# ishine/chunkformer

Hardware: AMD Instinct MI355X
Metric: audio-frames/sec (80-dim fbank) through encoder, chunkformer-large chunk=64, 1/2/4/8 GPU (higher is better)
Workload: dtype bf16

## Files before the change

chunkformer_amd/csrc/cfm_kernels.h:

```cpp
#pragma once
#include <hip/hip_runtime.h>
#include <stdint.h>

typedef __bf16 bf16;

#define CFM_HD_INLINE __host__ __device__ __forceinline__

namespace cfm {

int cu_count();

enum { EPI_STORE = 0, EPI_STORE_F32 = 1, EPI_RESID = 2, EPI_QKV = 3, EPI_GLU = 4, EPI_DW2 = 5 };
enum { ACT_NONE = 0, ACT_RELU = 1, ACT_SILU = 2, ACT_SILU_L2E = 3 };

struct EpiArgs {
  const float* bias = nullptr;
  float alpha = 1.f;
  void* out = nullptr;
  void* out2 = nullptr;
  int ldo = 0;
  int row_off = 0;
  float* x = nullptr;
  int ldx = 0;
  const uint8_t* rowmask = nullptr;
  int d = 0;
  int dk = 64;
  int col_group = 0;
  int store_mode = 0;
  int diag = 0;
  int wst = 1;
  int small_tiles = 0;
  int big_min_tiles = 0;
  int wsp_small_div = 1;
  int wsp_small_rows = 32768;
  int f16 = 0;
  const float* dw_w = nullptr;
  const float* dw_b = nullptr;
  int t2n = 0, t3n = 0;
};

int gemm_bf16_wst(int epi, int act, const bf16* A, int lda, const bf16* W, int ldw, int M, int N, int K,
                  const EpiArgs& ep, hipStream_t st);

enum { SITE_QKV = 1, SITE_OPROJ = 2, SITE_PW2 = 4, SITE_FFN2 = 8, SITE_FFN1 = 16, SITE_PW1 = 32, SITE_FE = 64 };

struct Tuning {
  int gemm_diag = 0, gemm_wst = 1, store_mode = 0, col_group = 0;
  int dw2_seg = 4;
  int fe_conv = 6;
  int fe_fuse_dw2 = 1;
  int nt_sites = 8;
  int big_min_tiles = 0;
  int wsp_small_div = 1;
  int wsp_small_rows = 32768;
  int attn_min_chunks = 2;
  void apply(EpiArgs& e, int site = 0) const {
    e.diag = gemm_diag;
    e.big_min_tiles = big_min_tiles;
    e.wsp_small_div = wsp_small_div;
    e.wsp_small_rows = wsp_small_rows;
    e.wst = gemm_wst;
    e.store_mode = (nt_sites & site) ? 2 : store_mode;
    e.col_group = col_group;
  }
};

template <typename T>
int gemm(int epi, int act, const T* A, int lda, const T* W, int ldw, int M, int N, int K, const EpiArgs& ep,
         hipStream_t st);

template <typename T>
inline int vocab_logits(const T* A, int rows, const T* W, const float* bias, int V, int d, float* out, int ldo,
                        hipStream_t st, const EpiArgs& tuned = EpiArgs()) {
  const int V1 = (sizeof(T) == 2 && V % 4 == 0) ? V / 256 * 256 : 0;
  if (V1 > 0) {
    EpiArgs e = tuned; e.bias = bias; e.out = out; e.ldo = ldo;
    if (const int r = gemm<T>(EPI_STORE_F32, ACT_NONE, A, d, W, d, rows, V1, d, e, st)) return r;
  }
  if (V1 < V) {
    EpiArgs e = tuned; e.bias = bias + V1; e.out = out + V1; e.ldo = ldo;
    if (const int r = gemm<T>(EPI_STORE_F32, ACT_NONE, A, d, W + (size_t)V1 * d, d, rows, V - V1, d, e, st)) return r;
  }
  return 0;
}
inline int logit_slab_rows(int V) {
  const size_t r = (((size_t)512 << 20) / ((size_t)V * sizeof(float))) / 256 * 256;
  return (int)(r < 256 ? 256 : r > 16384 ? 16384 : r);
}

template <typename T> struct ResidAdd {
  const T* y = nullptr;
  float alpha = 1.f;
  const uint8_t* ymask = nullptr;
  const T* y2 = nullptr;
  float alpha2 = 1.f;
  const uint8_t* ymask2 = nullptr;
  bool defer = false;
};
template <typename T>
int layernorm(float* x, const ResidAdd<T>& ra, int M, int d, const float* w, const float* b, float eps, T* out,
              const uint8_t* rowmask, hipStream_t st);
template <typename T>
int layernorm2(float* x, const ResidAdd<T>& ra, int M, int d, const float* w1, const float* b1, const float* w2,
               const float* b2, float eps, T* out, hipStream_t st);
template <typename T>
int layernorm2_f32(float* x, const ResidAdd<T>& ra, int M, int d, const float* w1, const float* b1, const float* w2,
                   const float* b2, float eps, float* out, hipStream_t st);

template <typename T>
int chunk_attention(const T* q, const T* kv, int kv_rows, const T* P, int p_rows, const float* pos_u,
                    const float* pos_v, const int32_t* desc, int nblk, int H, int dk, T* out, hipStream_t st,
                    int p_ld = 0);

CFM_HD_INLINE int qkv_kv_col(int cc, int which, int dk) { return (cc / dk) * 2 * dk + which * dk + (cc & (dk - 1)); }

int full_attention_bf16(const bf16* q, const bf16* kv, int kv_rows, const bf16* P, int p_rows, const float* pos_u,
                        const float* pos_v, const int32_t* desc, int nutt, int nd, int H, int dk, int t_keys,
                        bf16* out, hipStream_t st, int p_ld);
int chunk_attention_masked_bf16(const bf16* q, const bf16* kv, int kv_rows, const bf16* P, int p_rows,
                                const float* pos_u, const float* pos_v, const int32_t* desc, int n_chunks, int H,
                                int C, int W, bf16* out, hipStream_t st, int diag = 0, int p_ld = 0,
                                int min_chunks = 2);
int chunk_attention_masked_f16(const f16* q, const f16* kv, int kv_rows, const f16* P, int p_rows,
                               const float* pos_u, const float* pos_v, const int32_t* desc, int n_chunks, int H,
                               int C, int W, f16* out, hipStream_t st, int diag = 0, int p_ld = 0,
                               int min_chunks = 2);

bool attention_a128_eligible(int C, int W, int p_rows, int dk);
int vt_transpose_bf16(const bf16* kv, int kv_rows, int H, bf16* vt, int vt_ld, hipStream_t st);
int chunk_attention_masked_a128(const bf16* q, const bf16* kv, int kv_rows, const bf16* vt, int vt_ld, const bf16* P,
                                int p_rows, int p_ld, const float* pos_u, const float* pos_v, const int32_t* desc,
                                int n_chunks, int H, int C, int W, bf16* out, hipStream_t st);

template <typename T>
int conv_dw_ln_silu(const T* glu, const int32_t* desc, int nblk, int d, const float* wdw_t ,
                    const float* bdw, const float* lnw, const float* lnb, float eps, T* out, hipStream_t st);

template <typename T>
int frontend_conv0_dw(const float* feats, const float* const* tab, int step, const int32_t* meta, int meta_stride,
                      int nwin, int W,
                      const float* cmvn_mean, const float* cmvn_istd, const float* w0, const float* b0,
                      const float* w1, const float* b1, const float* wpack, const float* wfrag, int d, T* out,
                      hipStream_t st, int var = 1);
constexpr int FE_WPACK = 24;
constexpr int FE2_NFRAG = 23;
template <typename T>
int frontend_dw2(const T* in, int nwin, int T2, int d, const float* w, const float* b, T* out, hipStream_t st,
                 int seg = 4);

template <typename T>
int pos_table(int d, int p_rows, int anchor, T* out, hipStream_t st);
template <typename T>
int att_cache_in(const float* cache, int L, int row_elems, T* kv, hipStream_t st);
template <typename T>
int att_cache_out(const T* kv, int start_row, int L, int row_elems, float* cache, hipStream_t st);
template <typename T>
int att_cache_in_hl(const float* cache , int H, int L, int dk, T* kv, hipStream_t st);
template <typename T>
int att_cache_out_hl(const T* kv, int start_row, int H, int L, int dk, float* cache , hipStream_t st);
template <typename T>
int cnn_cache_in(const float* cache , int d, int lorder, T* glu, hipStream_t st);
template <typename T>
int cnn_cache_out(const T* glu, int start_row, int d, int lorder, float* cache, hipStream_t st);
template <typename T>
int cache_io(bool in, bool hl, float* acache, int H, int L, int dk, T* kv, float* ccache, int d, int lorder, T* glu,
             hipStream_t st);
int masks_from_plan(const int32_t* meta, int n, int C, int L, int R, uint8_t* att, uint8_t* pad, hipStream_t st);
bool ctc_argmax_eligible(int V, int d);
int ctc_argmax_bf16(const float* enc, int M, const bf16* W, const float* bias, int V, int d, int32_t* ids,
                    hipStream_t st);
int ctc_argmax_f16(const float* enc, int M, const f16* W, const float* bias, int V, int d, int32_t* ids,
                   hipStream_t st);
int ctc_collapse(const int32_t* ids, const int32_t* row_start, const int32_t* row_len, int B, int blank, int max_sil,
                 int32_t* tok, int32_t* tok_frame, int32_t* n_tok, int32_t* seg, int32_t* n_seg, hipStream_t st);
int log_softmax_rows(float* logits, int M, int V, int write_logp, int32_t* ids, hipStream_t st);
int ctc_topk_rows(const float* x, int M, int V, int k, int with_lse, float* vals, int32_t* ids, hipStream_t st);

}
```

chunkformer_amd/csrc/frontend.hip:

```cpp
#include <algorithm>
#include <cstdlib>
#include <type_traits>
#include "cfm_common.h"
#include "cfm_kernels.h"

namespace cfm {

constexpr int FE_T2_TILE = 8;
constexpr int FE_T1_ROWS = 2 * FE_T2_TILE + 1;
constexpr int FE_IN_ROWS = 2 * FE_T1_ROWS + 1;
constexpr int FE_F0 = 80, FE_F1 = 39, FE_F2 = 19, FE_F3 = 9;
constexpr int FE_CG = 16;

__device__ __forceinline__ const float* window_rows(const float* feats, const float* const* tab, int step,
                                                   const int32_t* m) {
  return tab ? tab[m[PM_UTT]] + (size_t)m[PM_CHUNK] * step * FE_F0 : feats + (size_t)m[PM_SRC_ROW] * FE_F0;
}

template <typename T>
__global__ __launch_bounds__(256) void fe_conv0_dw_kernel(const float* __restrict__ feats, const float* const* __restrict__ tab,
                                                          int step, const int32_t* __restrict__ meta,
                                                          int meta_stride, int W, int T2, const float* __restrict__ cm,
                                                          const float* __restrict__ ci, const float* __restrict__ w0,
                                                          const float* __restrict__ b0, const float* __restrict__ w1,
// ... 65 lines not shown
template <typename E, typename V>
CFM_DEV f32x16 mfma32x16(const V& a, const V& b, const f32x16& c) {
  if constexpr (std::is_same<E, f16>::value) return __builtin_amdgcn_mfma_f32_32x32x16_f16(a, b, c, 0, 0, 0);
  else return __builtin_amdgcn_mfma_f32_32x32x16_bf16(a, b, c, 0, 0, 0);
}
template <typename E>
__global__ __launch_bounds__(256, 3) void fe_conv0_dw_mfma_kernel(const float* __restrict__ feats,
                                                               const float* const* __restrict__ tab, int step,
                                                               const int32_t* __restrict__ meta, int meta_stride,
                                                               int W, int T2, const float* __restrict__ cm,
                                                               const float* __restrict__ ci,
                                                               const float* __restrict__ wpack, int d,
                                                               E* __restrict__ out) {
  typedef E ex8 __attribute__((ext_vector_type(8)));
  __shared__ float xin[FE_XROWS * FE_F0];
  constexpr int OPITCH = 144;
  __shared__ __attribute__((aligned(16))) char ostage[4][32 * OPITCH];
  const int tid = threadIdx.x;
  const int win = blockIdx.y;
  const int P = T2 * FE_F2;
  const int p0 = blockIdx.x * FE_POS_BLOCK;
  const int r0 = 4 * (p0 / FE_F2);
  const float* xsrc = window_rows(feats, tab, step, meta + (size_t)win * meta_stride);
  const int nvalid = min(meta[(size_t)win * meta_stride + PM_NVALID], W);
  for (int idx = tid; idx < FE_XROWS * FE_F0; idx += 256) {
    const int r = idx / FE_F0, f = idx - r * FE_F0, gr = r0 + r;
    float v = gr < nvalid ? xsrc[(size_t)gr * FE_F0 + f] : 0.f;
    if (cm) v = (v - cm[f]) * ci[f];
    xin[idx] = v;
  }
  __syncthreads();
  const int lane = tid & 63, wv = tid >> 6, hh = lane >> 5, n = lane & 31;
  const int pw = p0 + wv * 32;
  if (pw >= P) return;
  ex8 xa[9];
  {
    const int pos = min(pw + n, P - 1);
    const int t2 = pos / FE_F2, f2 = pos - t2 * FE_F2;
    const float* xb = xin + (4 * t2 - r0) * FE_F0 + 4 * f2;
#pragma unroll
    for (int s = 0; s < 9; ++s) {
      const float* xs = xb + 2 * (s / 3) * FE_F0 + 2 * (s % 3);
      if (hh == 0) {
#pragma unroll
        for (int j = 0; j < 8; ++j) xa[s][j] = (E)xs[(j / 3) * FE_F0 + j % 3];
      } else {
        xa[s][0] = (E)xs[2 * FE_F0 + 2];
        xa[s][1] = (E)1.f;
#pragma unroll
        for (int j = 2; j < 8; ++j) xa[s][j] = (E)0.f;
      }
    }
  }
  f32x4 qw[5];
  auto load_w = [&](int c) {
    const f32x4* wp = reinterpret_cast<const f32x4*>(wpack + (size_t)c * FE_WPACK);
#pragma unroll
    for (int i = 0; i < 5; ++i) qw[i] = wp[i];
  };
  load_w(n);
  const unsigned long long obase = (unsigned long long)(out + (size_t)win * P * d);
  const unsigned long long obu = ((unsigned long long)__builtin_amdgcn_readfirstlane((unsigned)(obase >> 32)) << 32) |
                                 (unsigned)__builtin_amdgcn_readfirstlane((unsigned)obase);
  const __amdgpu_buffer_rsrc_t ors = __builtin_amdgcn_make_buffer_rsrc(
      (void*)obu, (short)0, __builtin_amdgcn_readfirstlane(P * d * 2), 0x00020000);
  unsigned voff[4];
#pragma unroll
  for (int k = 0; k < 4; ++k) voff[k] = (unsigned)(((pw + (lane >> 3) + 8 * k) * d + (lane & 7) * 8) * 2);
  for (int ct = 0; ct < d; ct += 64) {
#pragma unroll
    for (int half = 0; half < 2; ++half) {
      const float t[9] = {qw[0][0], qw[0][1], qw[0][2], qw[0][3], qw[1][0], qw[1][1], qw[1][2], qw[1][3], qw[2][0]};
      ex8 wcur;
#pragma unroll
      for (int j = 0; j < 8; ++j) wcur[j] = (E)(hh ? (j == 0 ? t[8] : j == 1 ? qw[4][2] : 0.f) : t[j]);
      const float wkc[9] = {qw[2][1], qw[2][2], qw[2][3], qw[3][0], qw[3][1], qw[3][2], qw[3][3], qw[4][0], qw[4][1]};
      const f32x16 seed = {};
      f32x16 o;
#pragma unroll
      for (int r = 0; r < 16; ++r) o[r] = qw[4][3];
      load_w(min(ct + 32 * half + 32 + n, d - 1));
      f32x16 acc = mfma32x16<E>(xa[0], wcur, seed);
#pragma unroll
      for (int s = 0; s < 9; ++s) {
        f32x16 nxt;
        if (s + 1 < 9) nxt = mfma32x16<E>(xa[s + 1], wcur, seed);
        __builtin_amdgcn_sched_barrier(0);
#pragma unroll
        for (int r = 0; r < 16; ++r) o[r] = fmaf(fmaxf(acc[r], 0.f), wkc[s], o[r]);
        __builtin_amdgcn_sched_barrier(0);
        if (s + 1 < 9) acc = nxt;
      }
      char* os = ostage[wv];
#pragma unroll
      for (int r = 0; r < 16; ++r) {
        const int m = 8 * (r >> 2) + 4 * hh + (r & 3);
        *reinterpret_cast<E*>(os + m * OPITCH + (32 * half + n) * 2) = (E)o[r];
      }
    }
    const char* os = ostage[wv];
#pragma unroll
    for (int k = 0; k < 4; ++k) {
      const u32x4 v = *reinterpret_cast<const u32x4*>(os + ((lane >> 3) + 8 * k) * OPITCH + (lane & 7) * 16);
#ifndef CFM_FE_DIAG_NOSTORE
      __builtin_amdgcn_raw_buffer_store_b128(v, ors, voff[k], ct * 2, 0);
#else
      asm volatile("" ::"v"(v));
#endif
    }
  }
}

constexpr int FE2_WAVES = 4;
constexpr int FE2_POS = 256;
constexpr int FE2_T1ROWS = 2 * ((FE_F2 - 1 + FE2_POS - 1) / FE_F2) + 3;
constexpr int FE2_XROWS = 2 * FE2_T1ROWS + 1;
constexpr int FE2_SLOTS = (FE_F1 + 1) / 2;
__host__ __device__ constexpr int fe2_slot(int t1, int i) { return t1 * FE2_SLOTS + (t1 >> 1) * 11 + i; }
constexpr int FE2_PLANE = fe2_slot(FE2_T1ROWS - 1, FE2_SLOTS - 1) + 1;
constexpr int FE2_IMG = 2 * FE2_PLANE * 16;
constexpr int FE2_OPITCH = 80;
constexpr int FE2_NQ = FE2_XROWS * (FE_F0 / 4);
constexpr int FE2_NT = 64 * FE2_WAVES;
constexpr int FE2_QPT = (FE2_NQ + FE2_NT - 1) / FE2_NT;
typedef short short2v __attribute__((ext_vector_type(2)));
typedef float f32x2v __attribute__((ext_vector_type(2)));

template <typename E>
__device__ __forceinline__ unsigned fe2_relu_pk(float a, float b) {
  if constexpr (std::is_same<E, f16>::value) {
    typedef f16 h2v __attribute__((ext_vector_type(2)));
    short2v v = __builtin_bit_cast(short2v, __builtin_convertvector((f32x2v){a, b}, h2v));
    v = __builtin_elementwise_max(v, (short2v){0, 0});
    return __builtin_bit_cast(unsigned, v);
  }
  unsigned u;
  asm("v_cvt_pk_bf16_f32 %0, %1, %2 clamp" : "=v"(u) : "v"(a), "v"(b));
  return u;
}

template <typename E>
__device__ __forceinline__ bf16x8 pk8(float a, float b, float c, float d_, float e, float f, float g, float h) {
  typedef E e8v __attribute__((ext_vector_type(8)));
  return __builtin_bit_cast(bf16x8, (e8v){(E)a, (E)b, (E)c, (E)d_, (E)e, (E)f, (E)g, (E)h});
}
template <typename E>
__device__ __forceinline__ f32x16 fe2_mfma(const bf16x8& a, const bf16x8& b, const f32x16& c) {
  if constexpr (std::is_same<E, f16>::value)
    return __builtin_amdgcn_mfma_f32_32x32x16_f16(__builtin_bit_cast(f16x8, a), __builtin_bit_cast(f16x8, b), c, 0, 0, 0);
  else
    return __builtin_amdgcn_mfma_f32_32x32x16_bf16(a, b, c, 0, 0, 0);
}
template <typename E>
__global__ __launch_bounds__(FE2_NT, 2) void fe_conv0_dw_mfma2_kernel(const float* __restrict__ feats,
                                                                const float* const* __restrict__ tab, int step,
                                                                const int32_t* __restrict__ meta, int meta_stride,
                                                                int W, int T2, const float* __restrict__ cm,
                                                                const float* __restrict__ ci,
                                                                const float* __restrict__ wfrag, int d,
                                                                E* __restrict__ out) {
  __shared__ __attribute__((aligned(16))) char im2col[2 * FE2_IMG];
  constexpr int XBYTES = FE2_XROWS * FE_F0 * 4, OBYTES = FE2_WAVES * 32 * FE2_OPITCH;
  __shared__ __attribute__((aligned(16))) char xstage[XBYTES > OBYTES ? XBYTES : OBYTES];
  __shared__ __attribute__((aligned(16))) float cmvn[2][FE_F0];
  const int tid = threadIdx.x;
  const int lane = tid & 63, wv = tid >> 6, h = lane >> 5, n = lane & 31;
  if (cm && tid < 2 * FE_F0) cmvn[tid / FE_F0][tid % FE_F0] = (tid < FE_F0 ? cm : ci)[tid % FE_F0];
  const int win = blockIdx.z;
  const int P = T2 * FE_F2;
  const int ct = blockIdx.y * FE2_WAVES + wv;
  const bool active = ct * 32 < d;
  bf16x8 a0, a1[9][2];
  f32x16 seed;
  {
    const u32x4* fr = reinterpret_cast<const u32x4*>(wfrag) + (size_t)(active ? ct : 0) * FE2_NFRAG * 64 + lane;
    a0 = __builtin_bit_cast(bf16x8, fr[0]);
#pragma unroll
    for (int s = 0; s < 9; ++s)
#pragma unroll
      for (int t = 0; t < 2; ++t) a1[s][t] = __builtin_bit_cast(bf16x8, fr[(1 + 2 * s + t) * 64]);
#pragma unroll
    for (int i = 0; i < 4; ++i) {
      const f32x4 v = __builtin_bit_cast(f32x4, fr[(19 + i) * 64]);
#pragma unroll
      for (int r = 0; r < 4; ++r) seed[4 * i + r] = v[r];
    }
  }
  const float* xsrc = window_rows(feats, tab, step, meta + (size_t)win * meta_stride);
  const int nvalid = min(meta[(size_t)win * meta_stride + PM_NVALID], W);
  const int nck = (P + FE2_POS - 1) / FE2_POS;
  const int c_beg = (int)((long long)blockIdx.x * nck / gridDim.x), c_end = (int)((long long)(blockIdx.x + 1) * nck / gridDim.x);
  f32x4 pv[FE2_QPT];
  auto prefetch = [&](int c) {
    const int r0 = 4 * ((c * FE2_POS) / FE_F2);
#pragma unroll
    for (int i = 0; i < FE2_QPT; ++i) {
      const int q = tid + FE2_NT * i, r = q / (FE_F0 / 4), gr = r0 + r;
      pv[i] = (f32x4){0.f, 0.f, 0.f, 0.f};
      if (q < FE2_NQ && gr < nvalid)
        pv[i] = *reinterpret_cast<const f32x4*>(xsrc + (size_t)gr * FE_F0 + 4 * (q % (FE_F0 / 4)));
    }
  };
  if (c_beg < c_end) prefetch(c_beg);
  const unsigned long long obase = (unsigned long long)(out + (size_t)win * P * d);
  const unsigned long long obu = ((unsigned long long)__builtin_amdgcn_readfirstlane((unsigned)(obase >> 32)) << 32) |
                                 (unsigned)__builtin_amdgcn_readfirstlane((unsigned)obase);
  const __amdgpu_buffer_rsrc_t ors = __builtin_amdgcn_make_buffer_rsrc(
      (void*)obu, (short)0, __builtin_amdgcn_readfirstlane(P * d * 2), 0x00020000);
  char* sb = xstage + wv * 32 * FE2_OPITCH;
  const f32x16 zero = {};
  for (int c = c_beg; c < c_end; ++c) {
    const int p0 = c * FE2_POS, t2a = p0 / FE_F2;
    __syncthreads();
    {
      float* xs = reinterpret_cast<float*>(xstage);
#pragma unroll
      for (int i = 0; i < FE2_QPT; ++i) {
        const int q = tid + FE2_NT * i;
        if (q < FE2_NQ) {
          f32x4 x = pv[i];
          if (cm) {
            const int f = 4 * (q % (FE_F0 / 4));
            x = (x - *reinterpret_cast<const f32x4*>(&cmvn[0][f])) * *reinterpret_cast<const f32x4*>(&cmvn[1][f]);
          }
          *reinterpret_cast<f32x4*>(xs + 4 * q) = x;
        }
      }
    }
    __syncthreads();
    for (int idx = tid; idx < FE2_T1ROWS * FE2_SLOTS; idx += FE2_NT) {
      const int tl = idx / FE2_SLOTS, i = idx - tl * FE2_SLOTS;
      const float* xr = reinterpret_cast<const float*>(xstage) + (2 * tl) * FE_F0 + 4 * i;
      f32x4 A[3];
      float Ex[3];
#pragma unroll
      for (int a = 0; a < 3; ++a) {
        A[a] = *reinterpret_cast<const f32x4*>(xr + a * FE_F0);
        Ex[a] = i + 1 < FE2_SLOTS ? xr[a * FE_F0 + 4] : 0.f;
      }
      const bf16x8 lo0 = pk8<E>(A[0][0], A[0][1], A[0][2], A[1][0], A[1][1], A[1][2], A[2][0], A[2][1]);
      const bf16x8 hi0 = pk8<E>(A[2][2], 1.f, 0.f, 0.f, 0.f, 0.f, 0.f, 0.f);
      const int s0 = fe2_slot(tl, i) * 16, s1 = (FE2_PLANE + fe2_slot(tl, i)) * 16;
      *reinterpret_cast<bf16x8*>(im2col + s0) = lo0;
      *reinterpret_cast<bf16x8*>(im2col + FE2_IMG + s0) = hi0;
      if (2 * i + 1 < FE_F1) {
        const bf16x8 lo1 = pk8<E>(A[0][2], A[0][3], Ex[0], A[1][2], A[1][3], Ex[1], A[2][2], A[2][3]);
        const bf16x8 hi1 = pk8<E>(Ex[2], 1.f, 0.f, 0.f, 0.f, 0.f, 0.f, 0.f);
        *reinterpret_cast<bf16x8*>(im2col + s1) = lo1;
        *reinterpret_cast<bf16x8*>(im2col + FE2_IMG + s1) = hi1;
      }
    }
    __syncthreads();
    if (c + 1 < c_end) prefetch(c + 1);
    if (!active) continue;
    const int pend = min(p0 + FE2_POS, P);
    auto patch_base = [&](int pt) {
      const int pos = min(pt + n, P - 1);
      const int t2 = pos / FE_F2, f2 = pos - t2 * FE_F2;
      return im2col + h * FE2_IMG + (fe2_slot(2 * (t2 - t2a), 0) + f2) * 16;
    };
    auto tap_off = [](int s) { return (((s % 3) & 1) * FE2_PLANE + fe2_slot(s / 3, 0) + ((s % 3) >> 1)) * 16; };
    auto ld = [&](const char* xb, int s) { return *reinterpret_cast<const bf16x8*>(xb + tap_off(s)); };
    auto flush = [&](const char* sb, int pt) {
#pragma unroll
      for (int k = 0; k < 2; ++k) {
        const int pl = (lane >> 2) + 16 * k, ch = lane & 3;
        const u32x4 v = *reinterpret_cast<const u32x4*>(sb + pl * FE2_OPITCH + ch * 16);
#ifndef CFM_FE_DIAG_NOSTORE
        __builtin_amdgcn_raw_buffer_store_b128(v, ors, (unsigned)(((pt + pl) * d + ct * 32 + ch * 8) * 2), 0, 0);
#else
        asm volatile("" ::"v"(v));
#endif
      }
    };
    bf16x8 pb[9];
    {
      const char* xb = patch_base(p0);
#pragma unroll
      for (int s = 0; s < 9; ++s) pb[s] = ld(xb, s);
    }
    for (int pt = p0; pt < pend; pt += 32) {
      const char* xbn = patch_base(pt + 32 < pend ? pt + 32 : pt);
      f32x16 y = seed;
      f32x16 acc = fe2_mfma<E>(a0, pb[0], zero);
#pragma unroll
      for (int s = 0; s < 9; ++s) {
        f32x16 nxt;
        if (s + 1 < 9) nxt = fe2_mfma<E>(a0, pb[s + 1], zero);
        __builtin_amdgcn_sched_barrier(0);
        u32x4 r0, r1;
#pragma unroll
        for (int q = 0; q < 4; ++q) {
          r0[q] = fe2_relu_pk<E>(acc[2 * q], acc[2 * q + 1]);
          r1[q] = fe2_relu_pk<E>(acc[8 + 2 * q], acc[9 + 2 * q]);
        }
        y = fe2_mfma<E>(a1[s][0], __builtin_bit_cast(bf16x8, r0), y);
        y = fe2_mfma<E>(a1[s][1], __builtin_bit_cast(bf16x8, r1), y);
        if (s == 3) {
#pragma unroll
          for (int t = 0; t < 4; ++t) pb[t] = ld(xbn, t);
        }
        if (s == 7) {
#pragma unroll
          for (int t = 4; t < 9; ++t) pb[t] = ld(xbn, t);
        }
        __builtin_amdgcn_sched_barrier(0);
        if (s + 1 < 9) acc = nxt;
      }
#pragma unroll
      for (int g = 0; g < 4; ++g) {
        typedef E e2v __attribute__((ext_vector_type(2)));
        const e2v lo = __builtin_convertvector((f32x2v){y[4 * g], y[4 * g + 1]}, e2v);
        const e2v hi = __builtin_convertvector((f32x2v){y[4 * g + 2], y[4 * g + 3]}, e2v);
        const unsigned long long u = (unsigned long long)__builtin_bit_cast(unsigned, lo) |
                                     ((unsigned long long)__builtin_bit_cast(unsigned, hi) << 32);
        *reinterpret_cast<unsigned long long*>(sb + n * FE2_OPITCH + (8 * g + 4 * h) * 2) = u;
      }
      flush(sb, pt);
    }
  }
}

constexpr int FE_DW2_SEG = 4;
template <typename T>
__global__ __launch_bounds__(256) void fe_dw2_kernel(const T* __restrict__ in, int nwin, int T2, int T3, int d,
                                                     const float* __restrict__ w, const float* __restrict__ b,
                                                     T* __restrict__ out) {
  const int d8 = d >> 3;
  const size_t idx = (size_t)blockIdx.x * 256 + threadIdx.x;
  const size_t total = (size_t)nwin * FE_F3 * d8;
  if (idx >= total) return;
  const int t3a = (int)((long long)blockIdx.y * T3 / gridDim.y), t3b = (int)((long long)(blockIdx.y + 1) * T3 / gridDim.y);
  const int c = (int)(idx % d8) * 8;
  const size_t r = idx / d8;
  const int f3 = r % FE_F3;
  const size_t wn = r / FE_F3;
  if constexpr (sizeof(T) == 2 && DW2_DOT2) {
    constexpr int FMT = std::is_same<T, f16>::value ? 1 : 0;
    typedef unsigned u4_ __attribute__((ext_vector_type(4)));
    unsigned wd[9][8];
    float bias[8];
#pragma unroll
    for (int e = 0; e < 9; ++e)
#pragma unroll
      for (int q = 0; q < 8; ++q) wd[e][q] = dw2_wpack<FMT>(w[(size_t)e * d + c + q], q);
    load8(b + c, bias);
    const T* ib = in + (wn * T2 * FE_F2 + 2 * f3) * d + c;
    T* ob = out + (wn * T3 * FE_F3 + f3) * d + c;
    u4_ top[3];
#pragma unroll
    for (int v = 0; v < 3; ++v) top[v] = *reinterpret_cast<const u4_*>(ib + (size_t)(2 * t3a) * FE_F2 * d + (size_t)v * d);
    for (int t3 = t3a; t3 < t3b; ++t3) {
      u4_ mid[3], bot[3];
      const T* rb = ib + (size_t)(2 * t3 + 1) * FE_F2 * d;
#pragma unroll
      for (int v = 0; v < 3; ++v) {
        mid[v] = *reinterpret_cast<const u4_*>(rb + (size_t)v * d);
        bot[v] = *reinterpret_cast<const u4_*>(rb + (size_t)(FE_F2 + v) * d);
      }
      float a[8];
#pragma unroll
      for (int q = 0; q < 8; ++q) a[q] = bias[q];
#pragma unroll
      for (int v = 0; v < 3; ++v) {
        const u4_* rows[3] = {&top[v], &mid[v], &bot[v]};
#pragma unroll
        for (int i = 0; i < 3; ++i)
#pragma unroll
          for (int q = 0; q < 8; ++q) a[q] = dw2_dot<FMT>((*rows[i])[q >> 1], wd[3 * i + v][q], a[q]);
      }
      store8(ob + (size_t)t3 * FE_F3 * d, a);
#pragma unroll
      for (int v = 0; v < 3; ++v) top[v] = bot[v];
    }
    return;
  }
  float wt[9][8], bias[8];
#pragma unroll
  for (int e = 0; e < 9; ++e) load8(w + (size_t)e * d + c, wt[e]);
  load8(b + c, bias);
  const T* ib = in + (wn * T2 * FE_F2 + 2 * f3) * d + c;
  T* ob = out + (wn * T3 * FE_F3 + f3) * d + c;
  auto pin8 = [](float (&x)[8]) {
#pragma unroll
    for (int q = 0; q < 8; ++q) asm volatile("" : "+v"(x[q]));
  };
  float top[3][8];
#pragma unroll
  for (int v = 0; v < 3; ++v) {
    load8(ib + (size_t)(2 * t3a) * FE_F2 * d + (size_t)v * d, top[v]);
    pin8(top[v]);
  }
  for (int t3 = t3a; t3 < t3b; ++t3) {
    float mid[3][8], bot[3][8];
    const T* rb = ib + (size_t)(2 * t3 + 1) * FE_F2 * d;
#pragma unroll
    for (int v = 0; v < 3; ++v) {
      load8(rb + (size_t)v * d, mid[v]);
      load8(rb + (size_t)(FE_F2 + v) * d, bot[v]);
      pin8(mid[v]);
      pin8(bot[v]);
    }
    float a[8];
#pragma unroll
    for (int q = 0; q < 8; ++q) {
      float s = bias[q];
#pragma unroll
      for (int v = 0; v < 3; ++v) {
        s = fmaf(wt[v][q], top[v][q], s);
        s = fmaf(wt[3 + v][q], mid[v][q], s);
        s = fmaf(wt[6 + v][q], bot[v][q], s);
      }
      a[q] = s;
    }
    pin8(a);
    store8(ob + (size_t)t3 * FE_F3 * d, a);
#pragma unroll
    for (int v = 0; v < 3; ++v)
#pragma unroll
      for (int q = 0; q < 8; ++q) top[v][q] = bot[v][q];
  }
}

template <typename T>
int frontend_conv0_dw(const float* feats, const float* const* tab, int step, const int32_t* meta, int meta_stride,
                      int nwin, int W,
                      const float* cmvn_mean, const float* cmvn_istd, const float* w0, const float* b0,
                      const float* w1, const float* b1, const float* wpack, const float* wfrag, int d, T* out,
                      hipStream_t st, int var) {
  if (nwin <= 0) return 0;
  const int T1 = (W - 3) / 2 + 1, T2 = (T1 - 3) / 2 + 1;
  if (T2 <= 0 || d % FE_CG) return (int)hipErrorInvalidValue;
  const dim3 grid((T2 + FE_T2_TILE - 1) / FE_T2_TILE, nwin);
  if constexpr (sizeof(T) == 2) {
    if (d % 64 || (size_t)T2 * FE_F2 * d * sizeof(T) >= ((size_t)1 << 31)) return (int)hipErrorInvalidValue;
    if (var >= 2 && wfrag) {
      const int nck = (T2 * FE_F2 + FE2_POS - 1) / FE2_POS, nch = std::max(1, var - 1);
      const int nb = (nck + nch - 1) / nch;
      hipLaunchKernelGGL(fe_conv0_dw_mfma2_kernel<T>, dim3(nb, (d + 32 * FE2_WAVES - 1) / (32 * FE2_WAVES), nwin),
                         dim3(FE2_NT), 0, st, feats, tab, step,
                         meta, meta_stride, W, T2, cmvn_mean, cmvn_istd, wfrag, d, out);
      CFM_CHECK_LAUNCH();
      return 0;
    }
    if (var >= 1 || std::is_same<T, bf16>::value)
      hipLaunchKernelGGL(fe_conv0_dw_mfma_kernel<T>, dim3((T2 * FE_F2 + FE_POS_BLOCK - 1) / FE_POS_BLOCK, nwin), dim3(256),
                         0, st, feats, tab, step, meta, meta_stride, W, T2, cmvn_mean, cmvn_istd, wpack, d, out);
    else
      hipLaunchKernelGGL((fe_conv0_dw_kernel<T>), grid, dim3(256), 0, st, feats, tab, step, meta, meta_stride, W, T2,
                         cmvn_mean, cmvn_istd, w0, b0, w1, b1, d, out);
  } else {
    hipLaunchKernelGGL((fe_conv0_dw_kernel<T>), grid, dim3(256), 0, st, feats, tab, step, meta, meta_stride, W, T2,
                       cmvn_mean,
                       cmvn_istd, w0, b0, w1, b1, d, out);
  }
  CFM_CHECK_LAUNCH();
  return 0;
}

template <typename T>
// ... 28 lines not shown
```

chunkformer_amd/csrc/model.hip:

```cpp
#include <algorithm>
#include <cmath>
#include <cstdlib>
#include <cstring>
#include <map>
#include <memory>
#include <string>
#include <vector>

#include "../../include/cfm.h"
#include "../../include/cfm_ops.h"
#include "cfm_common.h"
#include "cfm_kernels.h"
#include "plan.h"
#include "status.h"
#include "workspace.h"

namespace cfm {

static thread_local std::string g_err;
cfm_status set_error(cfm_status s, const std::string& msg) {
  g_err = msg;
  return s;
}

// ... 392 lines not shown
        if (r == 0) return CFM_OK;
      }
    }
    if (wsb < ctc_ws_bytes(rows)) return set_error(CFM_ERR_VALUE, "ctc workspace too small");
    float* dst = nullptr;
    { const cfm_status hs = head_logits(enc, rows, logp, ws, st, &dst); if (hs != CFM_OK) return hs; }
    PROF(PC_CTC, log_softmax_rows(dst, rows, V, logp ? 1 : 0, ids, st));
    return CFM_OK;
  }

  cfm_status head_logits(const float* enc, int rows, float* logp, void* ws, hipStream_t st, float** out) const {
    const int d = cfg.d_model, V = cfg.vocab;
    Carver c(ws);
    float* logits = c.take<float>((size_t)rows * V);
    T* a = c.take<T>((size_t)rows * d);
    const T* A;
    if constexpr (sizeof(T) == 4) {
      A = reinterpret_cast<const T*>(enc);
    } else {
      KCHK(att_cache_in<T>(enc, rows, d, a, st));
      A = a;
    }
    float* dst = logp ? logp : logits;
    *out = dst;
    PROF(PC_CTC, vocab_logits<T>(A, rows, (const T*)fe.ctc_w, fe.ctc_b, V, d, dst, V, st, E()));
    return CFM_OK;
  }

  int topk_slab_rows() const override {
    return cfg.vocab <= 0 ? 0 : logit_slab_rows(cfg.vocab);
  }
  size_t ctc_topk_ws_bytes(int rows) const override { return ctc_ws_bytes(std::min(rows, topk_slab_rows())); }
  cfm_status ctc_topk(const float* enc, int rows, int k, float* vals, int32_t* ids, void* ws, size_t wsb,
                      hipStream_t st) const override {
    if (!fe.ctc_w) return set_error(CFM_ERR_ASSERT, "model has no CTC head (vocab == 0)");
    const int d = cfg.d_model, V = cfg.vocab, slab = topk_slab_rows();
    if (k < 1 || k > 16 || k > V) return set_error(CFM_ERR_VALUE, "top-k: 1 <= k <= 16 and k <= vocab");
    if (wsb < ctc_topk_ws_bytes(rows)) return set_error(CFM_ERR_VALUE, "ctc top-k workspace too small");
    for (int r0 = 0; r0 < rows; r0 += slab) {
      const int nr = std::min(slab, rows - r0);
      float* logits = nullptr;
      { const cfm_status hs = head_logits(enc + (size_t)r0 * d, nr, nullptr, ws, st, &logits); if (hs != CFM_OK) return hs; }
      PROF(PC_CTC, ctc_topk_rows(logits, nr, V, k, 1, vals + (size_t)r0 * k, ids + (size_t)r0 * k, st));
    }
    return CFM_OK;
  }
};

struct HostW {
  std::map<std::string, std::pair<const float*, int64_t>> m;
  const float* get(const std::string& k, int64_t numel) const {
    auto it = m.find(k);
    if (it == m.end()) throw std::string("missing weight " + k);
    if (it->second.second != numel)
      throw std::string("weight " + k + ": numel " + std::to_string(it->second.second) + " != " + std::to_string(numel));
    return it->second.first;
  }
  bool has(const std::string& k) const { return m.count(k) > 0; }
};

static uint16_t bf16_bits_rne(float f) {
  uint32_t u;
  std::memcpy(&u, &f, 4);
  if ((u & 0x7f800000u) == 0x7f800000u) return (uint16_t)((u >> 16) | ((u & 0xffff) ? 0x40 : 0));
  return (uint16_t)((u + 0x7fffu + ((u >> 16) & 1u)) >> 16);
}

template <typename T>
static cfm_status build_model(const cfm_config& cfg, const HostW& hw, int device, cfm_model** out) {
  auto* M = new ModelT<T>();
  std::unique_ptr<cfm_model> guard(M);
  M->cfg = cfg;
  M->device = device;
  const int d = cfg.d_model, ff = cfg.ffn_dim, H = cfg.n_heads, nb = cfg.num_blocks, V = cfg.vocab;
  struct Item { size_t off; size_t bytes; };
  std::vector<char> img;
  auto reserve = [&](size_t bytes) {
    size_t off = align_up(img.size());
    img.resize(off + align_up(bytes));
    return off;
  };
  std::vector<std::pair<size_t, void**>> fix;
  auto put_f32 = [&](const float* src, size_t n, float** slot) {
    size_t off = reserve(n * 4);
    std::memcpy(img.data() + off, src, n * 4);
    fix.push_back({off, (void**)slot});
  };
  auto put_T = [&](const std::vector<float>& src, void** slot) {
    size_t off = reserve(src.size() * sizeof(T));
    T* p = reinterpret_cast<T*>(img.data() + off);
    for (size_t i = 0; i < src.size(); ++i) {
      if constexpr (sizeof(T) == 4) p[i] = src[i];
      else if constexpr (std::is_same<T, f16>::value) p[i] = (f16)src[i];
      else {
        uint32_t u;
        std::memcpy(&u, &src[i], 4);
        uint16_t r;
        if ((u & 0x7f800000u) == 0x7f800000u) r = (uint16_t)((u >> 16) | ((u & 0xffff) ? 0x40 : 0));
        else r = (uint16_t)((u + 0x7fffu + ((u >> 16) & 1u)) >> 16);
        std::memcpy(&p[i], &r, 2);
      }
    }
    fix.push_back({off, slot});
  };
  auto vec = [&](const std::string& k, int64_t n) { const float* s = hw.get(k, n); return std::vector<float>(s, s + n); };
  try {
    const std::string E = "encoder.";
    FrontW& F = M->fe;
    if (cfg.has_cmvn) {
      put_f32(hw.get(E + "global_cmvn.mean", cfg.input_dim), cfg.input_dim, &F.cm);
      put_f32(hw.get(E + "global_cmvn.istd", cfg.input_dim), cfg.input_dim, &F.ci);
    }
    put_f32(hw.get(E + "embed.conv.0.weight", (int64_t)d * 9), (size_t)d * 9, &F.w0);
    put_f32(hw.get(E + "embed.conv.0.bias", d), d, &F.b0);
    put_f32(hw.get(E + "embed.conv.2.weight", (int64_t)d * 9), (size_t)d * 9, &F.w1);
    put_f32(hw.get(E + "embed.conv.2.bias", d), d, &F.b1);
    {
      const float *a = hw.get(E + "embed.conv.0.weight", (int64_t)d * 9), *ab = hw.get(E + "embed.conv.0.bias", d);
      const float *b = hw.get(E + "embed.conv.2.weight", (int64_t)d * 9), *bb = hw.get(E + "embed.conv.2.bias", d);
      std::vector<float> w((size_t)d * FE_WPACK, 0.f);
      for (int c = 0; c < d; ++c) {
        for (int e = 0; e < 9; ++e) {
          w[(size_t)c * FE_WPACK + e] = a[c * 9 + e];
          w[(size_t)c * FE_WPACK + 9 + e] = b[c * 9 + e];
        }
        w[(size_t)c * FE_WPACK + 18] = ab[c];
        w[(size_t)c * FE_WPACK + 19] = bb[c];
      }
      put_f32(w.data(), w.size(), &F.wpack);
      if (d % 32 == 0) {
        std::vector<uint32_t> fr((size_t)(d / 32) * FE2_NFRAG * 64 * 4, 0u);
        constexpr bool H16 = std::is_same<T, f16>::value;
        auto bf = [](float x) -> uint32_t {
          if constexpr (H16) {
            const f16 h = (f16)x;
            uint16_t u;
            std::memcpy(&u, &h, 2);
            return u;
          } else {
            return (uint32_t)bf16_bits_rne(x);
          }
        };
        const int sc0 = H16 ? 0 : -24, sc1 = H16 ? 0 : 24;
        for (int ct = 0; ct < d / 32; ++ct)
          for (int lane = 0; lane < 64; ++lane) {
            const int h = lane >> 5, n = lane & 31, c = ct * 32 + n;
            auto slot = [&](int q) { return &fr[(((size_t)ct * FE2_NFRAG + q) * 64 + lane) * 4]; };
            uint16_t a0[8];
            for (int j = 0; j < 8; ++j) {
              const int k = 8 * h + j;
              a0[j] = (uint16_t)bf(std::ldexp(k < 9 ? a[c * 9 + k] : k == 9 ? ab[c] : 0.f, sc0));
            }
            std::memcpy(slot(0), a0, 16);
            const bool own = h == ((n >> 2) & 1);
            const int town = n >> 4, j0 = (n & 3) + 4 * ((n >> 3) & 1);
            for (int sp = 0; sp < 9; ++sp)
              for (int t = 0; t < 2; ++t) {
                uint16_t a1[8] = {0, 0, 0, 0, 0, 0, 0, 0};
                if (own && t == town) a1[j0] = (uint16_t)bf(std::ldexp(b[c * 9 + sp], sc1));
                std::memcpy(slot(1 + 2 * sp + t), a1, 16);
              }
            for (int r = 0; r < 16; ++r) {
              const float v = bb[ct * 32 + (r & 3) + 8 * (r >> 2) + 4 * h];
              std::memcpy(slot(19 + r / 4) + (r & 3), &v, 4);
            }
          }
        put_f32(reinterpret_cast<const float*>(fr.data()), fr.size(), &F.wfrag);
      }
    }
    put_T(vec(E + "embed.conv.3.weight", (int64_t)d * d), &F.pw1);
    put_f32(hw.get(E + "embed.conv.3.bias", d), d, &F.b_pw1);
    {
      const float* s = hw.get(E + "embed.conv.5.weight", (int64_t)d * 9);
      std::vector<float> w((size_t)d * 9);
      for (int c = 0; c < d; ++c)
        for (int e = 0; e < 9; ++e) w[(size_t)e * d + c] = s[(size_t)c * 9 + e];
      put_f32(w.data(), w.size(), &F.w2);
    }
    put_f32(hw.get(E + "embed.conv.5.bias", d), d, &F.b2);
    put_T(vec(E + "embed.conv.6.weight", (int64_t)d * d), &F.pw2);
    put_f32(hw.get(E + "embed.conv.6.bias", d), d, &F.b_pw2);
    {
      const float* s = hw.get(E + "embed.out.weight", (int64_t)d * 9 * d);
      std::vector<float> w((size_t)d * 9 * d);
      for (int o = 0; o < d; ++o)
        for (int c = 0; c < d; ++c)
          for (int f = 0; f < 9; ++f) w[(size_t)o * 9 * d + f * d + c] = s[(size_t)o * 9 * d + c * 9 + f];
      put_T(w, &F.wout);
    }
    put_f32(hw.get(E + "embed.out.bias", d), d, &F.b_out);
    put_f32(hw.get(E + "after_norm.weight", d), d, &F.an_w);
    put_f32(hw.get(E + "after_norm.bias", d), d, &F.an_b);
    if (V > 0) {
      std::vector<float> w = vec("ctc.ctc_lo.weight", (int64_t)V * d);
      w.resize((size_t)(V + 63) / 64 * 64 * d, 0.f);
      put_T(w, &F.ctc_w);
      put_f32(hw.get("ctc.ctc_lo.bias", V), V, &F.ctc_b);
    }
    M->layers.resize(nb);
    for (int l = 0; l < nb; ++l) {
      LayerW& Lw = M->layers[l];
      const std::string p = E + "encoders." + std::to_string(l) + ".";
      auto scaled = [](std::vector<float> v, float f) { for (float& x : v) x *= f; return v; };
      const float s1 = kSiluPre<T> ? -kLog2e : 1.f, s2 = kSiluPre<T> ? -1.f / kLog2e : 1.f;
      put_T(scaled(vec(p + "feed_forward_macaron.w_1.weight", (int64_t)ff * d), s1), &Lw.ff1m);
      { const auto b = scaled(vec(p + "feed_forward_macaron.w_1.bias", ff), s1); put_f32(b.data(), b.size(), &Lw.b_ff1m); }
      put_T(scaled(vec(p + "feed_forward_macaron.w_2.weight", (int64_t)d * ff), s2), &Lw.ff2m);
      put_f32(hw.get(p + "feed_forward_macaron.w_2.bias", d), d, &Lw.b_ff2m);
      put_T(scaled(vec(p + "feed_forward.w_1.weight", (int64_t)ff * d), s1), &Lw.ff1);
      { const auto b = scaled(vec(p + "feed_forward.w_1.bias", ff), s1); put_f32(b.data(), b.size(), &Lw.b_ff1); }
      put_T(scaled(vec(p + "feed_forward.w_2.weight", (int64_t)d * ff), s2), &Lw.ff2);
      put_f32(hw.get(p + "feed_forward.w_2.bias", d), d, &Lw.b_ff2);
      {
        std::vector<float> w, b;
        for (const char* nm : {"linear_q", "linear_k", "linear_v"}) {
          auto wv = vec(p + "self_attn." + nm + ".weight", (int64_t)d * d);
          auto bv = vec(p + "self_attn." + nm + ".bias", d);
          w.insert(w.end(), wv.begin(), wv.end());
          b.insert(b.end(), bv.begin(), bv.end());
        }
        put_T(w, &Lw.qkv);
        put_f32(b.data(), b.size(), &Lw.b_qkv);
      }
      put_T(vec(p + "self_attn.linear_pos.weight", (int64_t)d * d), &Lw.pos);
      put_T(vec(p + "self_attn.linear_out.weight", (int64_t)d * d), &Lw.wo);
      put_f32(hw.get(p + "self_attn.linear_out.bias", d), d, &Lw.b_o);
      put_f32(hw.get(p + "self_attn.pos_bias_u", (int64_t)d), (size_t)d, &Lw.pu);
      put_f32(hw.get(p + "self_attn.pos_bias_v", (int64_t)d), (size_t)d, &Lw.pv);
      {
        const float* s = hw.get(p + "conv_module.pointwise_conv1.weight", (int64_t)2 * d * d);
        const float* sb = hw.get(p + "conv_module.pointwise_conv1.bias", 2 * d);
        std::vector<float> w((size_t)2 * d * d), b(2 * d);
        const float sg = kSiluPre<T> ? -kLog2e : 1.f;
        for (int t = 0; t < d / 16; ++t)
          for (int r = 0; r < 16; ++r) {
            const int ra = 16 * t + r, rg = d + 16 * t + r;
            std::memcpy(&w[(size_t)(32 * t + r) * d], s + (size_t)ra * d, 4 * d);
            for (int k = 0; k < d; ++k) w[(size_t)(32 * t + 16 + r) * d + k] = sg * s[(size_t)rg * d + k];
            b[32 * t + r] = sb[ra];
            b[32 * t + 16 + r] = sg * sb[rg];
          }
        put_T(w, &Lw.pw1);
        put_f32(b.data(), b.size(), &Lw.b_pw1);
      }
      {
        const float* s = hw.get(p + "conv_module.depthwise_conv.weight", (int64_t)d * 15);
        std::vector<float> w((size_t)15 * d);
        for (int c = 0; c < d; ++c)
          for (int t = 0; t < 15; ++t) w[(size_t)t * d + c] = s[c * 15 + t];
        put_f32(w.data(), w.size(), &Lw.dw_t);
      }
      put_f32(hw.get(p + "conv_module.depthwise_conv.bias", d), d, &Lw.b_dw);
      put_f32(hw.get(p + "conv_module.norm.weight", d), d, &Lw.cn_w);
      put_f32(hw.get(p + "conv_module.norm.bias", d), d, &Lw.cn_b);
      put_T(vec(p + "conv_module.pointwise_conv2.weight", (int64_t)d * d), &Lw.pw2);
      put_f32(hw.get(p + "conv_module.pointwise_conv2.bias", d), d, &Lw.b_pw2);
      const std::pair<const char*, float**> lns[] = {
          {"norm_ff_macaron.weight", &Lw.ln_ffm_w}, {"norm_ff_macaron.bias", &Lw.ln_ffm_b},
          {"norm_mha.weight", &Lw.ln_mha_w},        {"norm_mha.bias", &Lw.ln_mha_b},
          {"norm_conv.weight", &Lw.ln_conv_w},      {"norm_conv.bias", &Lw.ln_conv_b},
          {"norm_ff.weight", &Lw.ln_ff_w},          {"norm_ff.bias", &Lw.ln_ff_b},
          {"norm_final.weight", &Lw.ln_fin_w},      {"norm_final.bias", &Lw.ln_fin_b}};
      for (auto& kv : lns) put_f32(hw.get(p + kv.first, d), d, kv.second);
    }
    {
      std::vector<float> all((size_t)nb * d * d);
      for (int l = 0; l < nb; ++l) {
        const std::string p = E + "encoders." + std::to_string(l) + ".";
        std::memcpy(all.data() + (size_t)l * d * d, hw.get(p + "self_attn.linear_pos.weight", (int64_t)d * d),
                    (size_t)d * d * sizeof(float));
      }
      put_T(all, &F.pos_all);
    }
  } catch (const std::string& e) {
    return set_error(CFM_ERR_VALUE, e);
  }
  if (!cfg.has_cmvn) M->tune.fe_conv = 1;
  HIPC(hipSetDevice(device));
  HIPC(hipMalloc(&M->dev_mem, img.size()));
  HIPC(hipMemcpy(M->dev_mem, img.data(), img.size(), hipMemcpyHostToDevice));
  for (auto& f : fix) *f.second = (char*)M->dev_mem + f.first;
  *out = guard.release();
  return CFM_OK;
}

}

using namespace cfm;

extern "C" {

const char* cfm_version(void) { return "chunkformer_amd 0.1 (gfx950)"; }
const char* cfm_last_error(void) { return g_err.c_str(); }

cfm_status cfm_model_create(const cfm_config* cfg, const cfm_tensor_view* weights, int32_t n, int32_t device,
                            cfm_model** out) {
  if (!cfg || !out) return set_error(CFM_ERR_VALUE, "null argument");
  *out = nullptr;
  if (cfg->input_dim != 80) return set_error(CFM_ERR_ASSERT, "front-end kernel supports input_dim == 80");
  if (cfg->d_model != 128 && cfg->d_model != 256 && cfg->d_model != 512)
    return set_error(CFM_ERR_ASSERT, "d_model must be 128, 256 or 512");
  if (cfg->n_heads <= 0 || (cfg->d_model != 64 * cfg->n_heads && cfg->d_model != 128 * cfg->n_heads))
    return set_error(CFM_ERR_ASSERT, "head_dim (d_model / attention_heads) must be 64 or 128");
  if (cfg->ffn_dim % 128) return set_error(CFM_ERR_ASSERT, "ffn_dim must be a multiple of 128");
  if (cfg->kernel_size != 15) return set_error(CFM_ERR_ASSERT, "cnn_module_kernel must be 15");
  if (cfg->num_blocks <= 0 || cfg->vocab < 0) return set_error(CFM_ERR_VALUE, "bad num_blocks / vocab");
  HostW hw;
  for (int i = 0; i < n; ++i) hw.m[weights[i].name] = {weights[i].data, weights[i].numel};
  if (cfg->compute_dtype == CFM_DTYPE_F32) return build_model<float>(*cfg, hw, device, out);
  if (cfg->compute_dtype == CFM_DTYPE_BF16) return build_model<bf16>(*cfg, hw, device, out);
  if (cfg->compute_dtype == CFM_DTYPE_F16) return build_model<f16>(*cfg, hw, device, out);
  return set_error(CFM_ERR_VALUE, "unknown compute dtype");
}

void cfm_model_destroy(cfm_model* m) { delete m; }

cfm_status cfm_model_set_option(cfm_model* m, const char* key, int64_t value) {
// ... 265 lines not shown
```

Before: 32.13 million.

## Replace sparse per-tap MFMA depthwise accumulation with packed dot2 in frontend conv

The fused frontend conv0+depthwise kernel used to apply the 9 depthwise taps through 18 extra MFMAs whose A fragments were almost all zero (one nonzero per lane). It now packs pairs of tap weights per output element into 32-bit words on the host and accumulates with dot2 instructions on the ReLU'd conv0 outputs. Pairs of conv0 MFMAs are reissued to match. This removes wasted matrix-core work but moves the depthwise math onto the vector ALU and raises register use, since 80 packed weight words are kept per lane. The weight fragment layout grows from 23 to 25 slots.

```diff
diff --git a/chunkformer_amd/csrc/cfm_kernels.h b/chunkformer_amd/csrc/cfm_kernels.h
--- a/chunkformer_amd/csrc/cfm_kernels.h
+++ b/chunkformer_amd/csrc/cfm_kernels.h
@@ -143,7 +143,7 @@
                       const float* w1, const float* b1, const float* wpack, const float* wfrag, int d, T* out,
                       hipStream_t st, int var = 1);
 constexpr int FE_WPACK = 24;
-constexpr int FE2_NFRAG = 23;
+constexpr int FE2_NFRAG = 25;
 template <typename T>
 int frontend_dw2(const T* in, int nwin, int T2, int d, const float* w, const float* b, T* out, hipStream_t st,
                  int seg = 4);
diff --git a/chunkformer_amd/csrc/frontend.hip b/chunkformer_amd/csrc/frontend.hip
--- a/chunkformer_amd/csrc/frontend.hip
+++ b/chunkformer_amd/csrc/frontend.hip
@@ -241,6 +241,10 @@
     return __builtin_amdgcn_mfma_f32_32x32x16_bf16(a, b, c, 0, 0, 0);
 }
 template <typename E>
+__device__ __forceinline__ float fe2_dot2(unsigned x, unsigned w, float c) {
+  return dw2_dot<std::is_same<E, f16>::value ? 1 : 0>(x, w, c);
+}
+template <typename E>
 __global__ __launch_bounds__(FE2_NT, 2) void fe_conv0_dw_mfma2_kernel(const float* __restrict__ feats,
                                                                 const float* const* __restrict__ tab, int step,
                                                                 const int32_t* __restrict__ meta, int meta_stride,
@@ -259,18 +263,23 @@
   const int P = T2 * FE_F2;
   const int ct = blockIdx.y * FE2_WAVES + wv;
   const bool active = ct * 32 < d;
-  bf16x8 a0, a1[9][2];
+  bf16x8 a0;
+  unsigned wp[5][16];
   f32x16 seed;
   {
     const u32x4* fr = reinterpret_cast<const u32x4*>(wfrag) + (size_t)(active ? ct : 0) * FE2_NFRAG * 64 + lane;
     a0 = __builtin_bit_cast(bf16x8, fr[0]);
 #pragma unroll
-    for (int s = 0; s < 9; ++s)
-#pragma unroll
-      for (int t = 0; t < 2; ++t) a1[s][t] = __builtin_bit_cast(bf16x8, fr[(1 + 2 * s + t) * 64]);
+    for (int p = 0; p < 5; ++p)
+#pragma unroll
+      for (int i = 0; i < 4; ++i) {
+        const u32x4 v = fr[(1 + 4 * p + i) * 64];
+#pragma unroll
+        for (int r = 0; r < 4; ++r) wp[p][4 * i + r] = v[r];
+      }
 #pragma unroll
     for (int i = 0; i < 4; ++i) {
-      const f32x4 v = __builtin_bit_cast(f32x4, fr[(19 + i) * 64]);
+      const f32x4 v = __builtin_bit_cast(f32x4, fr[(21 + i) * 64]);
 #pragma unroll
       for (int r = 0; r < 4; ++r) seed[4 * i + r] = v[r];
     }
@@ -368,33 +377,36 @@
 #pragma unroll
       for (int s = 0; s < 9; ++s) pb[s] = ld(xb, s);
     }
+    f32x16 ca = fe2_mfma<E>(a0, pb[0], zero), cb = fe2_mfma<E>(a0, pb[1], zero);
     for (int pt = p0; pt < pend; pt += 32) {
       const char* xbn = patch_base(pt + 32 < pend ? pt + 32 : pt);
       f32x16 y = seed;
-      f32x16 acc = fe2_mfma<E>(a0, pb[0], zero);
-#pragma unroll
-      for (int s = 0; s < 9; ++s) {
-        f32x16 nxt;
-        if (s + 1 < 9) nxt = fe2_mfma<E>(a0, pb[s + 1], zero);
+#pragma unroll
+      for (int p = 0; p < 5; ++p) {
+        unsigned rp[16];
+#pragma unroll
+        for (int r = 0; r < 16; ++r) rp[r] = fe2_relu_pk<E>(ca[r], p < 4 ? cb[r] : 0.f);
         __builtin_amdgcn_sched_barrier(0);
-        u32x4 r0, r1;
-#pragma unroll
-        for (int q = 0; q < 4; ++q) {
-          r0[q] = fe2_relu_pk<E>(acc[2 * q], acc[2 * q + 1]);
-          r1[q] = fe2_relu_pk<E>(acc[8 + 2 * q], acc[9 + 2 * q]);
+        if (p < 3) {
+          ca = fe2_mfma<E>(a0, pb[2 * p + 2], zero);
+          cb = fe2_mfma<E>(a0, pb[2 * p + 3], zero);
+        } else if (p == 3) {
+          ca = fe2_mfma<E>(a0, pb[8], zero);
+        } else {
+          ca = fe2_mfma<E>(a0, pb[0], zero);
+          cb = fe2_mfma<E>(a0, pb[1], zero);
         }
-        y = fe2_mfma<E>(a1[s][0], __builtin_bit_cast(bf16x8, r0), y);
-        y = fe2_mfma<E>(a1[s][1], __builtin_bit_cast(bf16x8, r1), y);
-        if (s == 3) {
+#pragma unroll
+        for (int r = 0; r < 16; ++r) y[r] = fe2_dot2<E>(rp[r], wp[p][r], y[r]);
+        if (p == 1) {
 #pragma unroll
           for (int t = 0; t < 4; ++t) pb[t] = ld(xbn, t);
         }
-        if (s == 7) {
+        if (p == 3) {
 #pragma unroll
           for (int t = 4; t < 9; ++t) pb[t] = ld(xbn, t);
         }
         __builtin_amdgcn_sched_barrier(0);
-        if (s + 1 < 9) acc = nxt;
       }
 #pragma unroll
       for (int g = 0; g < 4; ++g) {
diff --git a/chunkformer_amd/csrc/model.hip b/chunkformer_amd/csrc/model.hip
--- a/chunkformer_amd/csrc/model.hip
+++ b/chunkformer_amd/csrc/model.hip
@@ -568,17 +568,14 @@
               a0[j] = (uint16_t)bf(std::ldexp(k < 9 ? a[c * 9 + k] : k == 9 ? ab[c] : 0.f, sc0));
             }
             std::memcpy(slot(0), a0, 16);
-            const bool own = h == ((n >> 2) & 1);
-            const int town = n >> 4, j0 = (n & 3) + 4 * ((n >> 3) & 1);
-            for (int sp = 0; sp < 9; ++sp)
-              for (int t = 0; t < 2; ++t) {
-                uint16_t a1[8] = {0, 0, 0, 0, 0, 0, 0, 0};
-                if (own && t == town) a1[j0] = (uint16_t)bf(std::ldexp(b[c * 9 + sp], sc1));
-                std::memcpy(slot(1 + 2 * sp + t), a1, 16);
+            for (int r = 0; r < 16; ++r) {
+              const int cr = ct * 32 + (r & 3) + 8 * (r >> 2) + 4 * h;
+              for (int p = 0; p < 5; ++p) {
+                const uint32_t lo = bf(std::ldexp(b[cr * 9 + 2 * p], sc1));
+                const uint32_t hi = 2 * p + 1 < 9 ? bf(std::ldexp(b[cr * 9 + 2 * p + 1], sc1)) : 0u;
+                slot(1 + 4 * p + r / 4)[r & 3] = lo | (hi << 16);
               }
-            for (int r = 0; r < 16; ++r) {
-              const float v = bb[ct * 32 + (r & 3) + 8 * (r >> 2) + 4 * h];
-              std::memcpy(slot(19 + r / 4) + (r & 3), &v, 4);
+              std::memcpy(slot(21 + r / 4) + (r & 3), &bb[cr], 4);
             }
           }
         put_f32(reinterpret_cast<const float*>(fr.data()), fr.size(), &F.wfrag);
```

After: 32.17 million (median of 6 runs). About the same (+0.1%).
